# Ulixes-8/UNet-Implementations

Hardware: AMD Instinct MI355X
Metric: images/sec (512x512, bs/GPU=8) Our_UNet train step (higher is better)
Workload: dtype f32; 1 GPU; Our_UNet 6-stage 3-class 512x512 bs=8/GPU fp32 train step (fwd + Dice/wCE loss + bwd + SGD-Nesterov), train mode, HIP conv/IN/upsample kernels; global_batch=8, parallelism=dp1, world=1

## Files before the change

### include/unet_hip.h

```cpp
#ifndef UNET_HIP_H_
#define UNET_HIP_H_

#include <stddef.h>
#include <stdint.h>

#ifdef __cplusplus
extern "C" {
#endif

#define UNET_ABI_VERSION 11

#define UNET_OK 0
#define UNET_E_INVALID (-1)
#define UNET_E_LAUNCH (-2)
#define UNET_E_WORKSPACE (-3)

typedef void* unet_stream_t;

const char* unet_last_error(void);
int unet_abi_version(void);
int unet_device_count(void);

int unet_debug_set_chunk_limit(int64_t bytes);

// ... 222 lines not shown
int unet_conv3x3_up_bwd_data(const float* D, const float* wd, int Cin_total, int ci_offset,
                             float* g, int N, int h, int w, int Cout, int Ccols, int accumulate,
                             unet_stream_t stream);

typedef struct unet_bwd_stats {
  const float* y;
  const float* mean;
  const float* rstd;
  const float* gamma;
  const float* beta;
  const float* mask;
  float slope;
  void* partial;
  size_t partial_bytes;
  int tiles_out;
} unet_bwd_stats;
int unet_conv3x3_bwd_data_bs(const float* dy, const float* wd, int Cin_total, int ci_offset,
                             float* dx, int N, int H, int W, int Cout, int Ccols, int stride,
                             int accumulate, unet_bwd_stats* bs, unet_stream_t stream);
int unet_conv3x3_bwd_data_bs_b16(const uint16_t* dy, const float* wd, int Cin_total, int ci_offset,
                                 uint16_t* dx, int N, int H, int W, int Cout, int Ccols, int stride,
                                 int accumulate, unet_bwd_stats* bs, unet_stream_t stream);
int unet_conv3x3_bwd_data_bs_bf16x3(const float* dy, const float* wd, const uint16_t* wd3,
                                    int Cin_total, int ci_offset, float* dx, int N, int H, int W,
                                    int Cout, int Ccols, int stride, int accumulate,
                                    unet_bwd_stats* bs, unet_stream_t stream);
int unet_conv3x3_up_bwd_data_bs(const float* D, const float* wd, int Cin_total, int ci_offset,
                                float* g, int N, int h, int w, int Cout, int Ccols, int accumulate,
                                unet_bwd_stats* bs, unet_stream_t stream);
int unet_conv_wino_supported(int N, int H, int W, int C0, int C1, int Cout);
int unet_set_c32_winograd(int on);
// ... 27 lines not shown
int unet_instnorm_lrelu_drop_bwd_partials(const float* ga, const float* y, const float* mean,
                                          const float* rstd, const float* gamma,
                                          const float* beta, const float* mask, float slope,
                                          float* dy, float* dgamma, float* dbeta, float* dbias,
                                          const void* partial, int tiles, void* workspace,
                                          size_t workspace_bytes, int N, int HW, int C,
                                          unet_stream_t stream);
int unet_instnorm_lrelu_drop_bwd_partials_b16(const uint16_t* ga, const uint16_t* y,
                                              const float* mean, const float* rstd,
                                              const float* gamma, const float* beta,
                                              const float* mask, float slope, uint16_t* dy,
                                              float* dgamma, float* dbeta, float* dbias,
                                              const void* partial, int tiles, void* workspace,
                                              size_t workspace_bytes, int N, int HW, int C,
                                              unet_stream_t stream);

int unet_conv_in_fwd_b16(const unet_act_src* s0, const unet_act_src* s1, float slope,
                         const float* w, const float* bias, int ksize, int stride, uint16_t* y,
                         void* workspace, size_t workspace_bytes, int* stats_px_out, int N, int H,
                         int W, int Cout, unet_stream_t stream);
int unet_conv_in_fwd_b16_wb(const unet_act_src* s0, const unet_act_src* s1, float slope,
                            const float* w, const uint16_t* wb, const float* bias, int ksize,
                            int stride, uint16_t* y, void* workspace, size_t workspace_bytes,
                            int* stats_px_out, int N, int H, int W, int Cout, unet_stream_t stream);
int unet_conv3x3_bwd_data_bs_b16_wb(const uint16_t* dy, const float* wd, const uint16_t* wdb,
                                    int Cin_total, int ci_offset, uint16_t* dx, int N, int H,
                                    int W, int Cout, int Ccols, int stride, int accumulate,
                                    unet_bwd_stats* bs, unet_stream_t stream);
int unet_conv_in_stats_finalize_b16(const uint16_t* y, void* workspace, size_t workspace_bytes,
                                    int stats_px, const float* gamma, const float* beta, float eps,
// ... 97 lines not shown
```

### unet-implementations_amd/_lib.py

```python
import ctypes
import os
import subprocess

_HERE = os.path.dirname(os.path.abspath(__file__))
LIB_PATH = os.environ.get("UNET_HIP_LIB") or os.path.join(_HERE, "libunet_hip.so")
CSRC = os.path.join(_HERE, "csrc")

ABI_VERSION = 11

_c = ctypes
_p = _c.c_void_p
_i = _c.c_int
_f = _c.c_float
_sz = _c.c_size_t
_i64 = _c.c_int64



class ActSrc(ctypes.Structure):
    _fields_ = [("x", _p), ("C", _i), ("alpha", _p), ("beta", _p)]


_ps = _c.POINTER(ActSrc)


class BwdStats(ctypes.Structure):
    _fields_ = [("y", _p), ("mean", _p), ("rstd", _p), ("gamma", _p), ("beta", _p), ("mask", _p),
                ("slope", _f), ("partial", _p), ("partial_bytes", _sz), ("tiles_out", _i)]


_pbs = _c.POINTER(BwdStats)

SIGNATURES = {
    "unet_last_error": (_c.c_char_p, []),
    "unet_abi_version": (_i, []),
    "unet_device_count": (_i, []),
    "unet_debug_set_chunk_limit": (_i, [_i64]),
    "unet_debug_record_launches": (_i, [_i]),
    "unet_debug_recorded_launches": (_sz, [_p, _sz]),
    "unet_nchw_to_nhwc": (_i, [_p, _p, _i, _i, _i, _i, _p]),
    "unet_nhwc_to_nchw": (_i, [_p, _p, _i, _i, _i, _i, _p]),
    "unet_pack_conv3x3_weights": (_i, [_p, _p, _p, _i, _i, _p]),
    "unet_conv3x3_fwd": (_i, [_p, _i, _p, _i, _p, _p, _p, _i, _i, _i, _i, _i, _p]),
# ... 74 lines not shown
    "unet_conv3x3_bwd_weight_is_winograd": (_i, [_i, _i, _i, _i, _i, _i]),
    "unet_conv_up_wino_supported": (_i, [_i, _i, _i, _i, _i, _i]),
    "unet_conv_up_in_fwd_wino": (_i, [_ps, _ps, _f, _p, _p, _p, _p, _sz, _c.POINTER(_i), _i, _i,
                                      _i, _i, _p]),
    "unet_conv3x3_bwd_data_bs_wino": (_i, [_p, _p, _i, _i, _p, _i, _i, _i, _i, _i, _pbs, _p]),
    "unet_conv3x3_bwd_data_bs_b16": (_i, [_p, _p, _i, _i, _p, _i, _i, _i, _i, _i, _i, _i, _pbs, _p]),
    "unet_conv3x3_bwd_data_bs_b16_wb": (_i, [_p, _p, _p, _i, _i, _p, _i, _i, _i, _i, _i, _i, _i, _pbs,
                                             _p]),
    "unet_conv3x3_bwd_data_bs_bf16x3": (_i, [_p, _p, _p, _i, _i, _p, _i, _i, _i, _i, _i, _i, _i, _pbs,
                                             _p]),
    "unet_conv3x3_up_bwd_data_bs": (_i, [_p, _p, _i, _i, _p, _i, _i, _i, _i, _i, _i, _pbs, _p]),
    "unet_instnorm_lrelu_drop_bwd_partials": (_i, [_p, _p, _p, _p, _p, _p, _p, _f, _p, _p, _p, _p,
                                                   _p, _i, _p, _sz, _i, _i, _i, _p]),
    "unet_instnorm_lrelu_drop_bwd_partials_b16": (_i, [_p, _p, _p, _p, _p, _p, _p, _f, _p, _p, _p, _p,
                                                       _p, _i, _p, _sz, _i, _i, _i, _p]),
    "unet_conv_in_fwd_b16": (_i, [_ps, _ps, _f, _p, _p, _i, _i, _p, _p, _sz, _c.POINTER(_i), _i, _i,
                                  _i, _i, _p]),
    "unet_conv_in_fwd_b16_wb": (_i, [_ps, _ps, _f, _p, _p, _p, _i, _i, _p, _p, _sz, _c.POINTER(_i),
                                     _i, _i, _i, _i, _p]),
    "unet_conv_in_stats_finalize_b16": (_i, [_p, _p, _sz, _i, _p, _p, _f, _p, _p, _p, _p, _p, _i, _i,
                                             _i, _p]),
    "unet_conv_in_bwd_weight_b16": (_i, [_ps, _f, _p, _p, _i, _i, _i, _i, _p, _sz, _i, _i, _i, _i,
                                         _p]),
    "unet_conv3x3_bwd_data_b16": (_i, [_p, _p, _i, _i, _p, _i, _i, _i, _i, _i, _i, _i, _p]),
    "unet_instnorm_lrelu_drop_bwd_b16": (_i, [_p, _p, _p, _p, _p, _p, _p, _f, _p, _p, _p, _p, _p,
                                              _sz, _i, _i, _i, _p]),
    "unet_upsample2x_in_fwd_b16": (_i, [_ps, _f, _p, _i, _i, _i, _p]),
    "unet_upsample2x_bwd_taps_b16": (_i, [_p, _p, _i, _i, _i, _i, _p]),
    "unet_conv3x3_up_bwd_weight_b16": (_i, [_ps, _f, _p, _p, _i, _i, _p, _sz, _i, _i, _i, _i, _p]),
    "unet_conv_up_in_fwd_b16_supported": (_i, [_i, _i, _i, _i, _i, _i]),
# ... 74 lines not shown
```

### unet-implementations_amd/csrc/common.h

```cpp
#pragma once
#include <hip/hip_runtime.h>
#include <stdarg.h>
#include <stdint.h>
#include <stdio.h>

#include "../../include/unet_hip.h"

typedef float f32x4 __attribute__((ext_vector_type(4)));
typedef float f32x16 __attribute__((ext_vector_type(16)));
typedef __bf16 bf16x8 __attribute__((ext_vector_type(8)));
typedef __bf16 bf16x4 __attribute__((ext_vector_type(4)));

void unet_set_error(const char* fmt, ...);

#define UNET_REQUIRE(cond, ...)        \
  do {                                 \
    if (!(cond)) {                     \
      unet_set_error(__VA_ARGS__);     \
      return UNET_E_INVALID;           \
    }                                  \
  } while (0)

#define UNET_CHECK_LAUNCH(name)                                              \
  do {                                                                       \
// ... 134 lines not shown
  }
  return v;
}

__device__ __forceinline__ void wf_merge(float& n, float& mean, float& m2, float nb, float mb,
                                         float m2b) {
  if (nb == 0.f) return;
  const float nt = n + nb;
  const float d = mb - mean;
  const float f = nb / nt;
  mean += d * f;
  m2 += m2b + d * d * n * f;
  n = nt;
}

#endif
```

### unet-implementations_amd/csrc/conv_igemm.hip

```cpp
#include "conv_params.h"

namespace unet_conv {
namespace {


template <int BM, int BN, int WM, int WN, int BK, bool FUSED = false, int KG = 1>
__global__ __launch_bounds__(256 * KG, KG == 1 ? 2 : 1) void conv_igemm_kernel(const IgemmParams p) {
  constexpr int LDA = BK + 4;
  constexpr int SEGS = BK / 4;
  constexpr int ROWS = 256 / SEGS;
  constexpr int TM = WM / 32, TN = WN / 32;
  constexpr int WAVES_N = BN / WN;
  static_assert((BM / WM) * (BN / WN) == 4, "4 waves per block");
  constexpr int A_PASSES = BM / ROWS;
  constexpr int B_PASSES = BN / ROWS;
  constexpr int A_TILE = BM * LDA, B_TILE = BN * LDA;
  extern __shared__ __attribute__((aligned(16))) float smem[];
  const int grp = KG > 1 ? __builtin_amdgcn_readfirstlane((int)(threadIdx.x >> 8)) : 0;
  const bool lead = KG == 1 || grp == 0;
  float* As = smem + grp * 2 * (A_TILE + B_TILE);
  float* Bs = As + 2 * A_TILE;

  const int tid = threadIdx.x & 255, lane = tid & 63, wave = tid >> 6;
  const int li = lane & 31, lh = lane >> 5;
// ... 1279 lines not shown

extern "C" int unet_conv3x3_fwd_bf16x3(const float* x0, int C0, const float* x1, int C1,
                                       const float* wf, const uint16_t* wf3, const float* bias,
                                       float* y, int N, int H, int W, int Cout, int stride,
                                       unet_stream_t stream) {
  return conv3x3_fwd_impl(x0, C0, x1, C1, wf, bias, y, N, H, W, Cout, stride, C0 == 3 ? 0 : 3,
                          (hipStream_t)stream, wf3);
}

static int conv3x3_bwd_data_impl(const float* dy, const float* wd, int Cin_total, int ci_offset,
                                 float* dx, int N, int H, int W, int Cout, int Ccols, int stride,
                                 int accumulate, int prec, hipStream_t stream,
                                 const uint16_t* wd3 = nullptr, int b16 = 0,
                                 unet_bwd_stats* bs = nullptr) {
  const long long es = b16 ? 2 : 4;
  if (bs) bs->tiles_out = 0;
  if (prec == 3 && bs && stride == 2) prec = 0;
  const bool use_bs = bs && (prec == 0 || prec == 3 || b16) && bs->y && bs->mean &&
                      bs->rstd && bs->gamma &&
                      bs->beta && bs->partial &&
                      bs->partial_bytes >= (size_t)N * ceil_div(H * W, 64) * Ccols * sizeof(float2);
  UNET_REQUIRE(dy && wd && dx, "conv3x3_bwd_data: null pointer");
  UNET_REQUIRE(prec != 3 || wd3, "conv3x3_bwd_data_bf16x3: the pre-split weight planes are null");
  UNET_REQUIRE(stride == 1 || stride == 2, "conv3x3_bwd_data: stride %d unsupported", stride);
  UNET_REQUIRE(Cout > 0 && Cout % 32 == 0 && Ccols > 0 && Ccols % 32 == 0 && ci_offset >= 0 &&
                   ci_offset + Ccols <= Cin_total,
               "conv3x3_bwd_data: bad channel counts Cout=%d Ccols=%d slice %d of %d", Cout, Ccols,
               ci_offset, Cin_total);
  UNET_REQUIRE(stride == 1 || (H % 2 == 0 && W % 2 == 0),
               "conv3x3_bwd_data: stride 2 needs even H, W");
// ... 59 lines not shown
    else if (rf_applicable(p) && (Cout == 32 || !patch_f32_applicable(p) || p.Hin % 8 != 0))
      rc = (Cout == 32) ? launch_igemm_rf<128, 32, 32, 32, true>(p, 1, stream, &bs_px)
                        : launch_igemm_rf<128, 32, 32, 32, false>(p, 1, stream, &bs_px);
    else
      rc = dispatch_igemm(p, stream, nullptr, use_bs ? &bs_px : nullptr);
    if (rc == UNET_OK && use_bs && bs_px > 0) bs->tiles_out = H * W / bs_px;
    return rc;
  }
  p.Hl = H / 2; p.Wl = W / 2; p.sout = 2;
  {
    const long long tiles = ceil_div64((long long)N * p.Hl * p.Wl, 128) * (Ccols / 32);
    if (prec == 0 && !b16) {
      IgemmParams q = p;
      if (!use_bs) q.bs_partial = nullptr;
      int bt = 0;
      const int rc = launch_dgrad_s2_patch_auto(q, stream, &bt);
      if (rc != 1) {
        if (rc == UNET_OK && use_bs && bt > 0) bs->tiles_out = bt;
        return rc;
      }
    }
    if (b16) {
      IgemmParams q = p;
      if (!use_bs) q.bs_partial = nullptr;
      int bt = 0;
      const int rc = launch_dgrad_s2_patch_b16_auto(q, stream, use_bs ? &bt : nullptr);
      if (rc != 1) {
        if (rc == UNET_OK && use_bs && bt > 0) bs->tiles_out = bt;
        return rc;
      }
      p.bs_partial = nullptr;
// ... 653 lines not shown
```

### unet-implementations_amd/csrc/conv_params.h

```cpp
#pragma once
#include "common.h"

namespace unet_conv {

struct IgemmParams {
  const float* src0;
  const float* src1;
  int C0, C1;
  const float* w;
  int tap_stride;
  int n_off;
  unsigned src0_bytes, src1_bytes, w_bytes;
  const float* bias;
  float* out;
  int ldo;
  int accumulate;
  int N, Hin, Win;
  int Hl, Wl;
  int Hout, Wout;
  int sin;
  int sout, py, px;
  int ntaps;
  unsigned tapw[3];
  int Ncols;
// ... 4 lines not shown
  const float* act1_alpha; const float* act1_beta;
  float slope;
  float2* stats;
  int stats_tiles;
  int tap_cstride;
  int src0_pitch;
  const float* bs_y;
  const float* bs_mean;
  const float* bs_rstd;
  const float* bs_gamma;
  const float* bs_beta;
  const float* bs_mask;
  float2* bs_partial;
  int bs_tiles;
  int bs_tile0;
};

long long& chunk_limit_bytes();
inline int batch_chunk(int N, long long per_image_bytes) {
  const long long lim = chunk_limit_bytes();
  const long long n = lim / (per_image_bytes > 0 ? per_image_bytes : 1);
  return (int)(n < N ? n : N);
}

inline void set_tap(IgemmParams& p, int t, int oy, int ox, int wt) {
  const unsigned e = (unsigned)(oy + 1) | ((unsigned)(ox + 1) << 2) | ((unsigned)wt << 4);
  p.tapw[t >> 2] |= e << ((t & 3) * 8);
}

#ifdef __HIPCC__
template <typename TO>
// ... 98 lines not shown
    }
  s1 += __shfl_xor(s1, 32, 64);
  s2 += __shfl_xor(s2, 32, 64);
  return float2{s1, s2};
}
template <int BN, int WAVES_M>
__device__ __forceinline__ bool block_col_sums(float2* red, float2& out) {
  __syncthreads();
  const int c = threadIdx.x;
  if (c >= BN) return false;
  float a = red[c].x, b = red[c].y;
#pragma unroll
  for (int k = 1; k < WAVES_M; ++k) { a += red[k * BN + c].x; b += red[k * BN + c].y; }
  out = float2{a, b};
  return true;
}

template <int BN, int WAVES_M>
__device__ __forceinline__ bool block_col_stats(float2* red, int wave_m, int col_local, bool writer,
                                                float2 mine, float cnt_wave, float2& out) {
  if (writer) red[wave_m * BN + col_local] = mine;
  __syncthreads();
  const int c = threadIdx.x;
  if (c >= BN) return false;
  float mean = red[c].x, m2 = red[c].y;
  if (WAVES_M == 2) {
    wf_merge_eq(mean, m2, red[BN + c].x, red[BN + c].y, cnt_wave);
  } else if (WAVES_M == 4) {
    float mean1 = red[2 * BN + c].x, m21 = red[2 * BN + c].y;
    wf_merge_eq(mean, m2, red[BN + c].x, red[BN + c].y, cnt_wave);
// ... 5 lines not shown
}
#endif

bool patch_f32_applicable(const IgemmParams& p);
int launch_patch_f32_auto(const IgemmParams& p, hipStream_t stream,
                          int* stats_px = nullptr, int* bs_px = nullptr);
int launch_patch_up_auto(const IgemmParams& p, hipStream_t stream, int* stats_px);
int& c32_winograd_flag();
bool c32_applicable(const IgemmParams& p);
int launch_c32(const IgemmParams& p, int fused, hipStream_t stream, int* tile_px);
bool wino_up32_applicable(const IgemmParams& p);
int launch_wino_up32(const IgemmParams& p, hipStream_t stream);
bool patch_s2_applicable(const IgemmParams& p);
int launch_patch_s2_auto(const IgemmParams& p, hipStream_t stream, int* stats_px);
int launch_patch_s2_b16_auto(const IgemmParams& p, hipStream_t stream, int* stats_px);
int launch_dgrad_s2_patch_auto(const IgemmParams& p, hipStream_t stream, int* bs_tiles_out);
int launch_patch_b16_up_auto(const IgemmParams& p, hipStream_t stream, int* stats_px);
int launch_dgrad_s2_patch_b16_auto(const IgemmParams& p, hipStream_t stream, int* bs_tiles_out);
int launch_patch_split_auto(const IgemmParams& p, hipStream_t stream);
int launch_patch_b16_auto(const IgemmParams& p, hipStream_t stream, int* stats_px,
                          int* bs_px = nullptr);
int launch_patch_split_fused_auto(const IgemmParams& p, hipStream_t stream, int* stats_px,
                                  int* bs_px);
bool patch_split_applicable(const IgemmParams& p);
int dispatch_igemm(const IgemmParams& p, hipStream_t stream,
                   int* stats_px = nullptr, int* bs_px = nullptr);
int dispatch_igemm_bf16(const IgemmParams& p, hipStream_t stream);
int dispatch_igemm_b16(const IgemmParams& p, hipStream_t stream, int* stats_px,
                       int* bs_px = nullptr);
int dispatch_igemm_split(const IgemmParams& p, hipStream_t stream);

// ... 2 lines not shown
```

### unet-implementations_amd/csrc/conv_patch.hip

```cpp
#include "conv_params.h"

#include <utility>

namespace unet_conv {
namespace {

template <int B, int... I, typename F>
__device__ __forceinline__ void for_range_p_impl(std::integer_sequence<int, I...>, F&& f) {
  (f(std::integral_constant<int, B + I>{}), ...);
}
template <int B, int E, typename F>
__device__ __forceinline__ void for_range_p(F&& f) {
  for_range_p_impl<B>(std::make_integer_sequence<int, (E > B ? E - B : 0)>{}, f);
}

template <int BN, int WM, int WN, int TH, bool ACT = false, bool STATS = false, bool BSTATS = false>
__global__ __launch_bounds__(256, 2) void conv_patch_split_kernel(const IgemmParams p) {
  constexpr int LDA = 24;
  constexpr int TW = 32, PW = TW + 2;
  constexpr int PPIX = (TH + 2) * PW;
  constexpr int P_PLANE = PPIX * LDA;
  constexpr int P_SLOTS = PPIX * 4;
  constexpr int P_PASSES = (P_SLOTS + 255) / 256;
  constexpr int B_SLOTS = BN * 6, B_PASSES = (B_SLOTS + 255) / 256;
// ... 1355 lines not shown
          }
        }
      }
  }
  if (p.bs_partial) {
    float2* red = reinterpret_cast<float2*>(Ps);
    static_assert(WAVES_M * BN * 2 <= PPIX * LDA, "reduction scratch fits in the patch area");
#pragma unroll
    for (int nb = 0; nb < TN; ++nb) {
      const float a = s1[nb] + __shfl_xor(s1[nb], 32, 64);
      const float b = s2[nb] + __shfl_xor(s2[nb], 32, 64);
      if (lh == 0) red[(wave / WAVES_N) * BN + wn0 + nb * 32 + li] = float2{a, b};
    }
    float2 out;
    if (block_col_sums<BN, WAVES_M>(red, out))
      p.bs_partial[((size_t)n * p.bs_tiles + ty * tiles_x + tx) * p.Ncols + n0 + tid] = out;
  }
}

template <int BN, int WM, int WN, int TH, bool WB = false>
__global__ __launch_bounds__(256, 2) void conv_dgrad_s2_patch_b16_kernel(const IgemmParams p) {
  constexpr int BK = 32, LDA = BK + 8;
  constexpr int TW = 32, PW = TW + 1, PH = TH + 1;
  constexpr int PPIX = PH * PW;
  constexpr int P_SLOTS = PPIX * 8;
  constexpr int P_PASSES = (P_SLOTS + 255) / 256;
  constexpr int B_SEGS = WB ? 4 : 8;
  constexpr int B_SETS = WB ? 2 : 1;
  constexpr int B_SLOTS = 3 * BN * B_SEGS, B_PASSES = (B_SLOTS + 255) / 256;
  constexpr int B_TILE = 3 * BN * LDA;
  constexpr int TM = WM / 32, TN = WN / 32;
// ... 585 lines not shown
  p.bs_tile0 = 0;
  if (!bs_tiles_out) p.bs_partial = nullptr;
  if (nc % 64 == 0 && p.Hl % 4 == 0 && pos / 128 * (nc / 64) >= 256) {
    p.bs_tiles = p.Hl * p.Wl / 128;
    if (bs_tiles_out) *bs_tiles_out = p.bs_partial ? p.bs_tiles : 0;
    return launch_dgrad_s2_patch_b16<64, 32, 64, 4>(p, stream);
  }
  if (nc == 32 && p.Hl % 8 == 0 && pos / 256 >= 256) {
    p.bs_tiles = p.Hl * p.Wl / 256;
    if (bs_tiles_out) *bs_tiles_out = p.bs_partial ? p.bs_tiles : 0;
    return launch_dgrad_s2_patch_b16<32, 64, 32, 8>(p, stream);
  }
  return 1;
}

int launch_dgrad_s2_patch_auto(const IgemmParams& p0, hipStream_t stream, int* bs_tiles_out) {
  IgemmParams p = p0;
  if (p.Wl % 32 != 0 || p.C0 % 32 != 0 || p.Hout != 2 * p.Hl || p.Wout != 2 * p.Wl) return 1;
  const long long pos = (long long)p.N * p.Hl * p.Wl;
  const int nc = p.Ncols;
  p.bs_tile0 = 0;
  if (nc % 64 == 0 && p.Hl % 4 == 0 && pos / 128 * (nc / 64) >= 256) {
    p.bs_tiles = p.Hl * p.Wl / 128;
    if (bs_tiles_out) *bs_tiles_out = p.bs_partial ? p.bs_tiles : 0;
    return launch_dgrad_s2_patch<64, 32, 64, 4>(p, stream);
  }
  if (nc == 32 && p.Hl % 8 == 0 && pos / 256 >= 256) {
    p.bs_tiles = p.Hl * p.Wl / 256;
    if (bs_tiles_out) *bs_tiles_out = p.bs_partial ? p.bs_tiles : 0;
    return launch_dgrad_s2_patch<32, 64, 32, 8>(p, stream);
  }
  return 1;
}

bool patch_s2_applicable(const IgemmParams& p) {
  IgemmParams std_taps{};
  for (int t = 0; t < 9; ++t) set_tap(std_taps, t, t / 3 - 1, t % 3 - 1, t);
  return p.ntaps == 9 && p.tap_cstride == 0 && p.src0_pitch == 0 && p.sin == 2 &&
         p.sout == 1 && p.Hin == 2 * p.Hl && p.Win == 2 * p.Wl && p.Hl == p.Hout &&
         p.Wl == p.Wout && p.Hl % 4 == 0 && p.Wl % 32 == 0 && p.C0 % 16 == 0 && p.C1 % 16 == 0 &&
         !p.accumulate && p.tapw[0] == std_taps.tapw[0] && p.tapw[1] == std_taps.tapw[1] &&
         p.tapw[2] == std_taps.tapw[2];
}

// ... 285 lines not shown
```

### unet-implementations_amd/csrc/conv_wino.hip

```cpp
#include "conv_params.h"
#include "lds_asm.h"
#include <utility>

namespace unet_conv {
namespace {

typedef int i32x4v __attribute__((ext_vector_type(4)));
template <int I> using wn_ic = std::integral_constant<int, I>;
template <int B, int... I, typename F>
__device__ __forceinline__ void wn_for_impl(std::integer_sequence<int, I...>, F&& f) {
  (f(wn_ic<B + I>{}), ...);
}
template <int B, int E, typename F>
__device__ __forceinline__ void wn_for(F&& f) {
  wn_for_impl<B>(std::make_integer_sequence<int, E - B>{}, f);
}

constexpr int WN_TH = 8, WN_TW = 32;
constexpr int WN_PW = WN_TW + 2, WN_PH = WN_TH + 2;
constexpr int WN_PPIX = WN_PH * WN_PW;
constexpr int WN_BN = 64;
constexpr int WN_KC = 8;
constexpr int WN_RP = 360;
constexpr int WN_BUF = 16 * 64 * WN_KC;
// ... 400 lines not shown
#pragma unroll
        for (int q = 0; q < 4; ++q) {
          const size_t pix = ((size_t)n * H + oy + (q >> 1)) * W + ox + 2 * r + (q & 1);
          const float y = p.bs_y[pix * p.ldo + col];
          const float z = fmaf(y, cf.A, cf.B0);
          const float gz = yv[b][r][q] * cf.mk * (z > 0.f ? 1.f : p.slope);
          s1 += gz;
          s2 = fmaf(gz, (y - cf.mu) * cf.rs, s2);
        }
      s1 += __shfl_xor(s1, 16, 64); s2 += __shfl_xor(s2, 16, 64);
      s1 += __shfl_xor(s1, 32, 64); s2 += __shfl_xor(s2, 32, 64);
      if (fk_e == 0) red[tg_e * WN_BN + 32 * nh_e + 16 * b + fm_e] = float2{s1, s2};
    }
    float2 out;
    if (block_col_sums<WN_BN, 4>(red, out))
      p.bs_partial[((size_t)n * p.bs_tiles + ty * tiles_x + tx) * p.Ncols + n0 + tid] = out;
  }
}

__device__ __forceinline__ void wino_pack_items(const float* __restrict__ w,
                                                float* __restrict__ uf, float* __restrict__ ud,
                                                int Cout, int Cin, int dir, long long block) {
  float* dst = dir == 0 ? uf : ud;
  if (!dst) return;
  const int Nn = dir == 0 ? Cout : Cin, Kt = dir == 0 ? Cin : Cout;
  const int kchunks = Kt / WN_KC;
  const long long items = (long long)Nn * kchunks;
  const long long idx = block * 256 + threadIdx.x;
  if (idx >= items) return;
  const int nl = (int)(idx & 63);
  const long long rest = idx >> 6;
// ... 179 lines not shown
               "conv3x3_bwd_data_bs_wino: bad channel slice");
  UNET_REQUIRE(wino_shape_ok(N, H, W, Cout, 0, Ccols, ci_offset),
               "conv3x3_bwd_data_bs_wino: shape N=%d %dx%d %d->%d not tiled by the Winograd kernel",
               N, H, W, Cout, Ccols);
  WinoParams wp{};
  IgemmParams& p = wp.g;
  p.src0 = dy; p.C0 = Cout; p.C1 = 0;
  p.src0_bytes = (unsigned)((long long)N * H * W * Cout * 4);
  p.n_off = ci_offset;
  p.out = dx; p.ldo = Ccols; p.N = N; p.Hin = p.Hl = p.Hout = H; p.Win = p.Wl = p.Wout = W;
  p.Ncols = Ccols;
  wp.wu = ud;
  const bool use_bs = bs && bs->y && bs->mean && bs->rstd && bs->gamma && bs->beta &&
                      bs->partial &&
                      bs->partial_bytes >= (size_t)N * (H * W / 256) * Ccols * sizeof(float2);
  if (bs) bs->tiles_out = 0;
  if (use_bs) {
    p.bs_y = bs->y; p.bs_mean = bs->mean; p.bs_rstd = bs->rstd; p.bs_gamma = bs->gamma;
    p.bs_beta = bs->beta; p.bs_mask = bs->mask; p.slope = bs->slope;
    p.bs_partial = reinterpret_cast<float2*>(bs->partial);
    p.bs_tiles = H * W / 256; p.bs_tile0 = 0;
    bs->tiles_out = p.bs_tiles;
    return launch_wino<false, false, true>(wp, (hipStream_t)stream);
  }
  return launch_wino<false, false, false>(wp, (hipStream_t)stream);
}
```

### unet-implementations_amd/csrc/instnorm.hip

```cpp
#include "common.h"

namespace {

constexpr int kThreads = 256;
constexpr int kColsumChunks = 32;

__host__ __device__ inline int split_for(int N, int HW, int C) {
  int ppi = kThreads / (C / 4);
  if (ppi < 1) ppi = 1;
  int max_split = HW / (ppi * 8);
  if (max_split < 1) max_split = 1;
  int want = (2048 + N - 1) / N;
  int s = want < max_split ? want : max_split;
  return s < 1 ? 1 : s;
}

template <typename TS>
__global__ __launch_bounds__(kThreads) void in_stats_kernel(const TS* __restrict__ y,
                                                            float2* __restrict__ partial, int HW,
                                                            int C, int split) {
  extern __shared__ __attribute__((aligned(16))) float smem[];
  const int lpp = C >> 2;
  const int groups = kThreads / lpp;
  const int tid = threadIdx.x;
// ... 47 lines not shown
  float* sm_m2 = sm_mean + groups * C;
  if (grp < groups) {
    sm_cnt[grp * lpp + c4] = cnt;
    *reinterpret_cast<f32x4*>(sm_mean + grp * C + c4 * 4) = mean;
    *reinterpret_cast<f32x4*>(sm_m2 + grp * C + c4 * 4) = m2;
  }
  __syncthreads();
  for (int c = tid; c < C; c += kThreads) {
    float n0 = 0.f, mu = 0.f, q = 0.f;
    for (int g = 0; g < groups; ++g)
      wf_merge(n0, mu, q, sm_cnt[g * lpp + (c >> 2)], sm_mean[g * C + c], sm_m2[g * C + c]);
    partial[((size_t)n * split + s) * C + c] = float2{mu, q};
  }
}

constexpr int FL = 32;
__global__ __launch_bounds__(32 * FL) void in_stats_finalize_kernel(
    const float2* __restrict__ partial, const float* __restrict__ gamma,
    const float* __restrict__ beta, float eps, const float* __restrict__ mask,
    float* __restrict__ mean, float* __restrict__ rstd, float* __restrict__ alpha,
    float* __restrict__ beta2, int N, int HW, int C, int split) {
  __shared__ float sn[FL][33], sm[FL][33], sq[FL][33];
  const int cl = threadIdx.x & 31, l = threadIdx.x >> 5;
  const int c = blockIdx.x * 32 + cl, n = blockIdx.y;
  const int per = (HW + split - 1) / split;
  float cnt = 0.f, mu = 0.f, q = 0.f;
  if (c < C) {
    for (int s = l; s < split; s += FL) {
      const int pb = s * per;
      int pe = pb + per;
      if (pe > HW) pe = HW;
// ... 206 lines not shown
  __syncthreads();
  for (int c = tid; c < C; c += kThreads) {
    float a = 0.f, b = 0.f;
    for (int g = 0; g < groups; ++g) {
      a += sm1[g * C + c];
      b += sm2[g * C + c];
    }
    partial[((size_t)n * split + s) * C + c] = float2{a, b};
  }
}

__global__ __launch_bounds__(32 * FL) void in_bwd_finalize1_kernel(const float2* __restrict__ partial,
                                                               float2* __restrict__ coef,
                                                               float2* __restrict__ sums, int HW,
                                                               int C, int split) {
  __shared__ double sa[FL][33], sb[FL][33];
  const int cl = threadIdx.x & 31, l = threadIdx.x >> 5;
  const int c = blockIdx.x * 32 + cl, n = blockIdx.y;
  double da_ = 0.0, db_ = 0.0;
  if (c < C)
    for (int s = l; s < split; s += FL) {
      const float2 v = partial[((size_t)n * split + s) * C + c];
      da_ += (double)v.x;
      db_ += (double)v.y;
    }
  sa[l][cl] = da_; sb[l][cl] = db_;
  __syncthreads();
  if (l == 0 && c < C) {
    da_ = 0.0; db_ = 0.0;
#pragma unroll 4
    for (int k = 0; k < FL; ++k) { da_ += sa[k][cl]; db_ += sb[k][cl]; }
    float a = (float)da_, b = (float)db_;
    const float inv = 1.f / (float)HW;
    coef[(size_t)n * C + c] = float2{a * inv, b * inv};
    sums[(size_t)n * C + c] = float2{a, b};
  }
}

template <typename TS>
__global__ __launch_bounds__(kThreads) void in_bwd_apply_kernel(
    const TS* ga , const TS* __restrict__ y, const float* __restrict__ mean,
    const float* __restrict__ rstd, const float* __restrict__ gamma,
    const float* __restrict__ beta, const float* __restrict__ mask, float slope,
    const float2* __restrict__ coef, TS* dy, float* __restrict__ dbias_partial,
    int HW, int C, int split, const float2* __restrict__ sums, float* __restrict__ dgamma,
    float* __restrict__ dbeta, float* __restrict__ dbias) {
  extern __shared__ __attribute__((aligned(16))) float smem[];
  const int lpp = C >> 2;
  const int groups = kThreads / lpp;
  const int tid = threadIdx.x;
  const int grp = tid / lpp, c4 = tid - grp * lpp;
// ... 197 lines not shown

extern "C" int unet_instnorm_lrelu_drop_bwd_partials_b16(
    const uint16_t* ga, const uint16_t* y, const float* mean, const float* rstd,
    const float* gamma, const float* beta, const float* mask, float slope, uint16_t* dy,
    float* dgamma, float* dbeta, float* dbias, const void* partial, int tiles, void* workspace,
    size_t workspace_bytes, int N, int HW, int C, unet_stream_t stream) {
  UNET_REQUIRE(partial && tiles > 0, "instnorm_lrelu_drop_bwd_partials_b16: no summaries");
  return instnorm_bwd_impl<__bf16>(reinterpret_cast<const __bf16*>(ga),
                                   reinterpret_cast<const __bf16*>(y), mean, rstd, gamma, beta,
                                   mask, slope, reinterpret_cast<__bf16*>(dy), dgamma, dbeta, dbias,
                                   workspace, workspace_bytes, N, HW, C, (hipStream_t)stream,
                                   reinterpret_cast<const float2*>(partial), tiles);
}

template <typename TS>
static int instnorm_bwd_impl(const TS* ga, const TS* y, const float* mean, const float* rstd,
                             const float* gamma, const float* beta, const float* mask, float slope,
                             TS* dy, float* dgamma, float* dbeta, float* dbias, void* workspace,
                             size_t workspace_bytes, int N, int HW, int C, hipStream_t stream,
                             const float2* ext_partial, int ext_tiles) {
  UNET_REQUIRE(ga && y && mean && rstd && gamma && beta && dy && workspace,
               "instnorm_lrelu_drop_bwd: null pointer");
  UNET_REQUIRE(shape_ok(N, HW, C) && kThreads % (C / 4) == 0,
               "instnorm_lrelu_drop_bwd: unsupported shape N=%d HW=%d C=%d", N, HW, C);
  if (workspace_bytes < unet_instnorm_workspace_bytes(N, HW, C)) {
    unet_set_error("instnorm_lrelu_drop_bwd: workspace too small");
    return UNET_E_WORKSPACE;
  }
  const int split = split_for(N, HW, C);
  const int groups = kThreads / (C / 4);
// ... 31 lines not shown
```

### unet-implementations_amd/ops.py

```python
import ctypes
import functools
import struct
import threading

import torch

from ._lib import ActSrc, BwdStats, check, lib


_raw_stream = getattr(torch._C, "_cuda_getCurrentRawStream", None)
_raw_device = getattr(torch._C, "_cuda_getDevice", None)


def _stream():
    if _raw_stream is not None and _raw_device is not None:
        return _raw_stream(_raw_device())
    return torch.cuda.current_stream().cuda_stream


class KernelTimer:

    def __init__(self, only=None):
        self.only = only
        self.records = []
# ... 84 lines not shown
    return getattr(lib(), name)


@functools.lru_cache(maxsize=None)
def _twin(name, b16):
    return getattr(lib(), name + "_b16" if b16 else name)


def _call_nxt(fn, args, nxt):
    if nxt is None:
        check(fn(*args, None, _stream()))
        return
    bs = nxt.c_struct()
    check(fn(*args, ctypes.byref(bs), _stream()))
    nxt.tiles = bs.tiles_out


_defer = threading.local()


def _wgrad_ws(nbytes, like):
    ws = _ws(nbytes, like)
    held = getattr(_defer, "held", None)
    if held is not None:
        held.append(ws)
    return ws


class wgrad_deferral:

# ... 172 lines not shown
    assert wf.shape[0] == 9 and wf.shape[2] == C0 + C1
    Ho, Wo = (H - 1) // stride + 1, (W - 1) // stride + 1
    y = out if out is not None else _f32((N, Ho, Wo, Cout), x0)
    fn, planes, tag = _sel_conv3x3_fwd(_prec(bf16), C0)
    if planes and wf3 is None:
        raise ValueError("bf16x3 needs wf3 from pack_conv3x3_weights_bf16x3")
    w3 = (_ptr(wf3),) if planes else ()
    t0 = _begin("conv")
    check(fn(_ptr(x0), C0, _ptr(x1), C1, _ptr(wf), *w3, _ptr(bias), _ptr(y), N, H, W, Cout, stride,
             _stream()))
    if t0 is not None:
        _timer.end(tag, 2.0 * N * Ho * Wo * 9 * (C0 + C1) * Cout, 1, t0)
    return y


class NextNorm:

    __slots__ = ("y", "st", "gamma", "beta", "mask", "slope", "partial", "tiles")

    def __init__(self, y, st, gamma, beta, mask, slope):
        self.y, self.st, self.gamma, self.beta, self.mask, self.slope = y, st, gamma, beta, mask, slope
        self.partial, self.tiles = None, 0

    def c_struct(self):
        N, H, W, C = self.y.shape
        nbytes = N * ((H * W + 63) // 64) * C * 8
        self.partial = torch.empty(nbytes, dtype=torch.uint8, device=self.y.device)
        return BwdStats(_ptr(self.y), _ptr(self.st[0]), _ptr(self.st[1]), _ptr(self.gamma),
                        _ptr(self.beta), _ptr(self.mask), self.slope, _ptr(self.partial), nbytes, 0)


def _c32_winograd(N, H, W, Cin, Cout, stride):
    return bool(lib().unet_conv_c32_is_winograd(N, H, W, Cin, Cout, stride))


_c32_override = None


def c32_winograd_override():
    return _c32_override


class c32_winograd_scope:

# ... 126 lines not shown
    check(lib().unet_instnorm_stats(_ptr(y), _ptr(gamma), _ptr(beta), eps, _ptr(st[0]),
                                    _ptr(st[1]), _ptr(st[2]), _ptr(st[3]), _ptr(ws), ws.numel(), N,
                                    H * W, C, _stream()))
    return st


def instnorm_lrelu_drop_fwd(y, alpha, beta2, mask, slope, out=None):
    N, H, W, C = y.shape
    a = out if out is not None else torch.empty_like(y)
    check(lib().unet_instnorm_lrelu_drop_fwd(_ptr(y), _ptr(alpha), _ptr(beta2), _ptr(mask), slope,
                                             _ptr(a), N, H * W, C, _stream()))
    return a


def instnorm_lrelu_drop_bwd(ga, y, mean, rstd, gamma, beta, mask, slope, dgamma, dbeta, dbias,
                            out=None, partials=None):
    N, H, W, C = y.shape
    dy = ga if out is None else out
    ws = _ws(lib().unet_instnorm_workspace_bytes(N, H * W, C), y)
    if partials is not None:
        name, part, launches, passes = "unet_instnorm_lrelu_drop_bwd_partials", \
            (_ptr(partials[0]), partials[1]), 2, 3.0
    else:
        name, part, launches, passes = "unet_instnorm_lrelu_drop_bwd", (), 5, 5
        if _is_b16(y) != _is_b16(ga):
            raise TypeError("ga and y must share their storage type")
    t0 = _begin()
    check(_twin(name, _is_b16(y))(
        _ptr(ga), _ptr(y), _ptr(mean), _ptr(rstd), _ptr(gamma), _ptr(beta), _ptr(mask), slope,
        _ptr(dy), _ptr(dgamma), _ptr(dbeta), _ptr(dbias), *part, _ptr(ws), ws.numel(), N, H * W, C,
        _stream()))
    if t0 is not None:
        _timer.end("instnorm_bwd", 0.0, launches, t0, nbytes=y.element_size() * passes * y.numel())
    return dy
# ... 664 lines not shown
```

Baseline: 468.7 images/s.

## Finalize instance-norm backward partial sums inside the dgrad kernel via last-workgroup counter

The stride-2 patch dgrad and Winograd dgrad kernels now store per-tile IN backward partial sums with atomic stores. The last workgroup per column block, found through an atomic ticket counter, reduces those partials into coef/sums inside the same kernel. The IN backward then runs a single apply kernel instead of a separate finalize launch plus apply. This removes one kernel launch and one pass over the partials per norm layer, at the cost of a persistent counter buffer, extra LDS and a serialized reduction in the last workgroup.

```diff
diff --git a/include/unet_hip.h b/include/unet_hip.h
--- a/include/unet_hip.h
+++ b/include/unet_hip.h
@@ -260,7 +260,12 @@
   void* partial;
   size_t partial_bytes;
   int tiles_out;
+  void* coef;
+  void* counters;
+  size_t counters_bytes;
+  int finalized_out;
 } unet_bwd_stats;
+#define UNET_BWD_STATS_FINALIZE 0x46494e31
 int unet_conv3x3_bwd_data_bs(const float* dy, const float* wd, int Cin_total, int ci_offset,
                              float* dx, int N, int H, int W, int Cout, int Ccols, int stride,
                              int accumulate, unet_bwd_stats* bs, unet_stream_t stream);
@@ -318,6 +323,19 @@
                                               const void* partial, int tiles, void* workspace,
                                               size_t workspace_bytes, int N, int HW, int C,
                                               unet_stream_t stream);
+int unet_instnorm_lrelu_drop_bwd_finalized(const float* ga, const float* y, const float* mean,
+                                           const float* rstd, const float* gamma,
+                                           const float* beta, const float* mask, float slope,
+                                           float* dy, float* dgamma, float* dbeta, float* dbias,
+                                           const void* coef_sums, int N, int HW, int C,
+                                           unet_stream_t stream);
+int unet_instnorm_lrelu_drop_bwd_finalized_b16(const uint16_t* ga, const uint16_t* y,
+                                               const float* mean, const float* rstd,
+                                               const float* gamma, const float* beta,
+                                               const float* mask, float slope, uint16_t* dy,
+                                               float* dgamma, float* dbeta, float* dbias,
+                                               const void* coef_sums, int N, int HW, int C,
+                                               unet_stream_t stream);
 
 int unet_conv_in_fwd_b16(const unet_act_src* s0, const unet_act_src* s1, float slope,
                          const float* w, const float* bias, int ksize, int stride, uint16_t* y,
diff --git a/unet-implementations_amd/_lib.py b/unet-implementations_amd/_lib.py
--- a/unet-implementations_amd/_lib.py
+++ b/unet-implementations_amd/_lib.py
@@ -26,7 +26,8 @@
 
 class BwdStats(ctypes.Structure):
     _fields_ = [("y", _p), ("mean", _p), ("rstd", _p), ("gamma", _p), ("beta", _p), ("mask", _p),
-                ("slope", _f), ("partial", _p), ("partial_bytes", _sz), ("tiles_out", _i)]
+                ("slope", _f), ("partial", _p), ("partial_bytes", _sz), ("tiles_out", _i),
+                ("coef", _p), ("counters", _p), ("counters_bytes", _sz), ("finalized_out", _i)]
 
 
 _pbs = _c.POINTER(BwdStats)
@@ -131,6 +132,10 @@
                                                    _p, _i, _p, _sz, _i, _i, _i, _p]),
     "unet_instnorm_lrelu_drop_bwd_partials_b16": (_i, [_p, _p, _p, _p, _p, _p, _p, _f, _p, _p, _p, _p,
                                                        _p, _i, _p, _sz, _i, _i, _i, _p]),
+    "unet_instnorm_lrelu_drop_bwd_finalized": (_i, [_p, _p, _p, _p, _p, _p, _p, _f, _p, _p, _p, _p,
+                                                    _p, _i, _i, _i, _p]),
+    "unet_instnorm_lrelu_drop_bwd_finalized_b16": (_i, [_p, _p, _p, _p, _p, _p, _p, _f, _p, _p, _p,
+                                                        _p, _p, _i, _i, _i, _p]),
     "unet_conv_in_fwd_b16": (_i, [_ps, _ps, _f, _p, _p, _i, _i, _p, _p, _sz, _c.POINTER(_i), _i, _i,
                                   _i, _i, _p]),
     "unet_conv_in_fwd_b16_wb": (_i, [_ps, _ps, _f, _p, _p, _p, _i, _i, _p, _p, _sz, _c.POINTER(_i),
diff --git a/unet-implementations_amd/csrc/common.h b/unet-implementations_amd/csrc/common.h
--- a/unet-implementations_amd/csrc/common.h
+++ b/unet-implementations_amd/csrc/common.h
@@ -172,4 +172,76 @@
   n = nt;
 }
 
+__device__ __forceinline__ void st_summary(float2* dst, const float2 v) {
+  const unsigned long long bits =
+      ((unsigned long long)__float_as_uint(v.y) << 32) | (unsigned long long)__float_as_uint(v.x);
+  __hip_atomic_store(reinterpret_cast<unsigned long long*>(dst), bits, __ATOMIC_RELAXED,
+                     __HIP_MEMORY_SCOPE_AGENT);
+}
+template <bool COHERENT>
+__device__ __forceinline__ float2 ld_summary(const float2* src) {
+  if constexpr (COHERENT) {
+    const unsigned long long bits =
+        __hip_atomic_load(reinterpret_cast<const unsigned long long*>(src), __ATOMIC_RELAXED,
+                          __HIP_MEMORY_SCOPE_AGENT);
+    return float2{__uint_as_float((unsigned)bits), __uint_as_float((unsigned)(bits >> 32))};
+  } else {
+    return *src;
+  }
+}
+__device__ __forceinline__ bool finalize_by_last_workgroup(unsigned* counter, unsigned expected,
+                                                           unsigned* flag, int writers) {
+  if ((int)threadIdx.x < writers) asm volatile("s_waitcnt vmcnt(0)" ::: "memory");
+  __syncthreads();
+  if (threadIdx.x == 0) {
+    const unsigned ticket =
+        __hip_atomic_fetch_add(counter, 1u, __ATOMIC_RELAXED, __HIP_MEMORY_SCOPE_AGENT);
+    const bool last = ticket + 1u == expected;
+    if (last) __hip_atomic_store(counter, 0u, __ATOMIC_RELAXED, __HIP_MEMORY_SCOPE_AGENT);
+    *flag = last ? 1u : 0u;
+  }
+  __syncthreads();
+  const bool last = *flag != 0u;
+  __builtin_amdgcn_fence(__ATOMIC_ACQUIRE, "wavefront");
+  return last;
+}
+
+constexpr int kFinLanes = 32;
+template <int T, bool COHERENT>
+__device__ __forceinline__ void in_bwd_finalize1_body(const float2* partial, float2* coef,
+                                                      float2* sums, int HW, int C, int split,
+                                                      int n, int cg, double* sa, double* sb) {
+  const int cl = threadIdx.x & 31;
+  const int c = cg * 32 + cl;
+  for (int l = threadIdx.x >> 5; l < kFinLanes; l += T / 32) {
+    double da_ = 0.0, db_ = 0.0;
+    if (c < C)
+      for (int s = l; s < split; s += 4 * kFinLanes) {
+        float2 v[4];
+#pragma unroll
+        for (int j = 0; j < 4; ++j)
+          if (s + j * kFinLanes < split)
+            v[j] = ld_summary<COHERENT>(partial + ((size_t)n * split + s + j * kFinLanes) * C + c);
+#pragma unroll
+        for (int j = 0; j < 4; ++j)
+          if (s + j * kFinLanes < split) {
+            da_ += (double)v[j].x;
+            db_ += (double)v[j].y;
+          }
+      }
+    sa[l * 32 + cl] = da_; sb[l * 32 + cl] = db_;
+  }
+  __syncthreads();
+  if (threadIdx.x < 32 && c < C) {
+    double da_ = 0.0, db_ = 0.0;
+#pragma unroll 4
+    for (int k = 0; k < kFinLanes; ++k) { da_ += sa[k * 32 + cl]; db_ += sb[k * 32 + cl]; }
+    float a = (float)da_, b = (float)db_;
+    const float inv = 1.f / (float)HW;
+    coef[(size_t)n * C + c] = float2{a * inv, b * inv};
+    sums[(size_t)n * C + c] = float2{a, b};
+  }
+  __syncthreads();
+}
+
 #endif
diff --git a/unet-implementations_amd/csrc/conv_igemm.hip b/unet-implementations_amd/csrc/conv_igemm.hip
--- a/unet-implementations_amd/csrc/conv_igemm.hip
+++ b/unet-implementations_amd/csrc/conv_igemm.hip
@@ -1317,6 +1317,7 @@
                                  const uint16_t* wd3 = nullptr, int b16 = 0,
                                  unet_bwd_stats* bs = nullptr) {
   const long long es = b16 ? 2 : 4;
+  unet_bwd_stats* const bs_fin = bs_finalize_requested(bs);
   if (bs) bs->tiles_out = 0;
   if (prec == 3 && bs && stride == 2) prec = 0;
   const bool use_bs = bs && (prec == 0 || prec == 3 || b16) && bs->y && bs->mean &&
@@ -1406,7 +1407,7 @@
       IgemmParams q = p;
       if (!use_bs) q.bs_partial = nullptr;
       int bt = 0;
-      const int rc = launch_dgrad_s2_patch_auto(q, stream, &bt);
+      const int rc = launch_dgrad_s2_patch_auto(q, stream, &bt, use_bs ? bs_fin : nullptr);
       if (rc != 1) {
         if (rc == UNET_OK && use_bs && bt > 0) bs->tiles_out = bt;
         return rc;
diff --git a/unet-implementations_amd/csrc/conv_params.h b/unet-implementations_amd/csrc/conv_params.h
--- a/unet-implementations_amd/csrc/conv_params.h
+++ b/unet-implementations_amd/csrc/conv_params.h
@@ -42,7 +42,29 @@
   float2* bs_partial;
   int bs_tiles;
   int bs_tile0;
+  unsigned* bs_counter;
+  float2* bs_coef;
+  float2* bs_sums;
+  int bs_HW;
 };
+
+constexpr int kFinalizeInKernelMaxTiles = 256;
+
+inline unet_bwd_stats* bs_finalize_requested(unet_bwd_stats* bs) {
+  return bs && bs->tiles_out == UNET_BWD_STATS_FINALIZE ? bs : nullptr;
+}
+inline void bs_finalize_setup(IgemmParams& p, unet_bwd_stats* bs, int HW, int BN) {
+  p.bs_counter = nullptr;
+  if (bs) bs->finalized_out = 0;
+  if (!bs || !p.bs_partial || !bs->coef || !bs->counters) return;
+  if (p.bs_tiles < 1 || p.bs_tiles > kFinalizeInKernelMaxTiles || p.Ncols % BN) return;
+  if (bs->counters_bytes < (size_t)p.N * (p.Ncols / BN) * sizeof(unsigned)) return;
+  p.bs_counter = reinterpret_cast<unsigned*>(bs->counters);
+  p.bs_coef = reinterpret_cast<float2*>(bs->coef);
+  p.bs_sums = p.bs_coef + (size_t)p.N * p.Ncols;
+  p.bs_HW = HW;
+  bs->finalized_out = 1;
+}
 
 long long& chunk_limit_bytes();
 inline int batch_chunk(int N, long long per_image_bytes) {
@@ -171,6 +193,23 @@
   for (int k = 1; k < WAVES_M; ++k) { a += red[k * BN + c].x; b += red[k * BN + c].y; }
   out = float2{a, b};
   return true;
+}
+
+constexpr size_t kBsFinalizeLds = 16 + 2 * kFinLanes * 32 * sizeof(double);
+template <int T, int BN>
+__device__ __forceinline__ void bs_finalize_in_kernel(const IgemmParams& p, int n, int n0,
+                                                      void* lds) {
+  if (!p.bs_counter) return;
+  unsigned* flag = reinterpret_cast<unsigned*>(lds);
+  double* sa = reinterpret_cast<double*>(reinterpret_cast<char*>(lds) + 16);
+  double* sb = sa + kFinLanes * 32;
+  if (!finalize_by_last_workgroup(p.bs_counter + (size_t)n * (p.Ncols / BN) + n0 / BN,
+                                  (unsigned)p.bs_tiles, flag, BN))
+    return;
+#pragma unroll 1
+  for (int g = 0; g < BN / 32; ++g)
+    in_bwd_finalize1_body<T, true>(p.bs_partial, p.bs_coef, p.bs_sums, p.bs_HW, p.Ncols,
+                                   p.bs_tiles, n, n0 / 32 + g, sa, sb);
 }
 
 template <int BN, int WAVES_M>
@@ -206,7 +245,8 @@
 bool patch_s2_applicable(const IgemmParams& p);
 int launch_patch_s2_auto(const IgemmParams& p, hipStream_t stream, int* stats_px);
 int launch_patch_s2_b16_auto(const IgemmParams& p, hipStream_t stream, int* stats_px);
-int launch_dgrad_s2_patch_auto(const IgemmParams& p, hipStream_t stream, int* bs_tiles_out);
+int launch_dgrad_s2_patch_auto(const IgemmParams& p, hipStream_t stream, int* bs_tiles_out,
+                               unet_bwd_stats* bs = nullptr);
 int launch_patch_b16_up_auto(const IgemmParams& p, hipStream_t stream, int* stats_px);
 int launch_dgrad_s2_patch_b16_auto(const IgemmParams& p, hipStream_t stream, int* bs_tiles_out);
 int launch_patch_split_auto(const IgemmParams& p, hipStream_t stream);
diff --git a/unet-implementations_amd/csrc/conv_patch.hip b/unet-implementations_amd/csrc/conv_patch.hip
--- a/unet-implementations_amd/csrc/conv_patch.hip
+++ b/unet-implementations_amd/csrc/conv_patch.hip
@@ -1393,7 +1393,9 @@
     }
     float2 out;
     if (block_col_sums<BN, WAVES_M>(red, out))
-      p.bs_partial[((size_t)n * p.bs_tiles + ty * tiles_x + tx) * p.Ncols + n0 + tid] = out;
+      st_summary(p.bs_partial + ((size_t)n * p.bs_tiles + ty * tiles_x + tx) * p.Ncols + n0 + tid, out);
+    static_assert(kBsFinalizeLds <= PPIX * LDA * sizeof(float), "finalize scratch fits in the patch area");
+    bs_finalize_in_kernel<256, BN>(p, n, n0, smem);
   }
 }
 
@@ -2009,7 +2011,8 @@
   return 1;
 }
 
-int launch_dgrad_s2_patch_auto(const IgemmParams& p0, hipStream_t stream, int* bs_tiles_out) {
+int launch_dgrad_s2_patch_auto(const IgemmParams& p0, hipStream_t stream, int* bs_tiles_out,
+                               unet_bwd_stats* bs) {
   IgemmParams p = p0;
   if (p.Wl % 32 != 0 || p.C0 % 32 != 0 || p.Hout != 2 * p.Hl || p.Wout != 2 * p.Wl) return 1;
   const long long pos = (long long)p.N * p.Hl * p.Wl;
@@ -2018,11 +2021,13 @@
   if (nc % 64 == 0 && p.Hl % 4 == 0 && pos / 128 * (nc / 64) >= 256) {
     p.bs_tiles = p.Hl * p.Wl / 128;
     if (bs_tiles_out) *bs_tiles_out = p.bs_partial ? p.bs_tiles : 0;
+    bs_finalize_setup(p, bs, p.Hout * p.Wout, 64);
     return launch_dgrad_s2_patch<64, 32, 64, 4>(p, stream);
   }
   if (nc == 32 && p.Hl % 8 == 0 && pos / 256 >= 256) {
     p.bs_tiles = p.Hl * p.Wl / 256;
     if (bs_tiles_out) *bs_tiles_out = p.bs_partial ? p.bs_tiles : 0;
+    bs_finalize_setup(p, bs, p.Hout * p.Wout, 32);
     return launch_dgrad_s2_patch<32, 64, 32, 8>(p, stream);
   }
   return 1;
diff --git a/unet-implementations_amd/csrc/conv_wino.hip b/unet-implementations_amd/csrc/conv_wino.hip
--- a/unet-implementations_amd/csrc/conv_wino.hip
+++ b/unet-implementations_amd/csrc/conv_wino.hip
@@ -438,7 +438,8 @@
     }
     float2 out;
     if (block_col_sums<WN_BN, 4>(red, out))
-      p.bs_partial[((size_t)n * p.bs_tiles + ty * tiles_x + tx) * p.Ncols + n0 + tid] = out;
+      st_summary(p.bs_partial + ((size_t)n * p.bs_tiles + ty * tiles_x + tx) * p.Ncols + n0 + tid, out);
+    bs_finalize_in_kernel<512, WN_BN>(p, n, n0, smem);
   }
 }
 
@@ -648,6 +649,7 @@
   const bool use_bs = bs && bs->y && bs->mean && bs->rstd && bs->gamma && bs->beta &&
                       bs->partial &&
                       bs->partial_bytes >= (size_t)N * (H * W / 256) * Ccols * sizeof(float2);
+  unet_bwd_stats* const bs_fin = bs_finalize_requested(bs);
   if (bs) bs->tiles_out = 0;
   if (use_bs) {
     p.bs_y = bs->y; p.bs_mean = bs->mean; p.bs_rstd = bs->rstd; p.bs_gamma = bs->gamma;
@@ -655,6 +657,7 @@
     p.bs_partial = reinterpret_cast<float2*>(bs->partial);
     p.bs_tiles = H * W / 256; p.bs_tile0 = 0;
     bs->tiles_out = p.bs_tiles;
+    bs_finalize_setup(p, bs_fin, H * W, WN_BN);
     return launch_wino<false, false, true>(wp, (hipStream_t)stream);
   }
   return launch_wino<false, false, false>(wp, (hipStream_t)stream);
diff --git a/unet-implementations_amd/csrc/instnorm.hip b/unet-implementations_amd/csrc/instnorm.hip
--- a/unet-implementations_amd/csrc/instnorm.hip
+++ b/unet-implementations_amd/csrc/instnorm.hip
@@ -85,7 +85,7 @@
   }
 }
 
-constexpr int FL = 32;
+constexpr int FL = kFinLanes;
 __global__ __launch_bounds__(32 * FL) void in_stats_finalize_kernel(
     const float2* __restrict__ partial, const float* __restrict__ gamma,
     const float* __restrict__ beta, float eps, const float* __restrict__ mask,
@@ -322,27 +322,9 @@
                                                                float2* __restrict__ coef,
                                                                float2* __restrict__ sums, int HW,
                                                                int C, int split) {
-  __shared__ double sa[FL][33], sb[FL][33];
-  const int cl = threadIdx.x & 31, l = threadIdx.x >> 5;
-  const int c = blockIdx.x * 32 + cl, n = blockIdx.y;
-  double da_ = 0.0, db_ = 0.0;
-  if (c < C)
-    for (int s = l; s < split; s += FL) {
-      const float2 v = partial[((size_t)n * split + s) * C + c];
-      da_ += (double)v.x;
-      db_ += (double)v.y;
-    }
-  sa[l][cl] = da_; sb[l][cl] = db_;
-  __syncthreads();
-  if (l == 0 && c < C) {
-    da_ = 0.0; db_ = 0.0;
-#pragma unroll 4
-    for (int k = 0; k < FL; ++k) { da_ += sa[k][cl]; db_ += sb[k][cl]; }
-    float a = (float)da_, b = (float)db_;
-    const float inv = 1.f / (float)HW;
-    coef[(size_t)n * C + c] = float2{a * inv, b * inv};
-    sums[(size_t)n * C + c] = float2{a, b};
-  }
+  __shared__ double sa[FL * 32], sb[FL * 32];
+  in_bwd_finalize1_body<32 * FL, false>(partial, coef, sums, HW, C, split, blockIdx.y, blockIdx.x,
+                                        sa, sb);
 }
 
 template <typename TS>
@@ -570,6 +552,50 @@
 }
 
 template <typename TS>
+static int instnorm_bwd_apply_impl(const TS* ga, const TS* y, const float* mean, const float* rstd,
+                                   const float* gamma, const float* beta, const float* mask,
+                                   float slope, TS* dy, float* dgamma, float* dbeta, float* dbias,
+                                   const void* coef_sums, int N, int HW, int C,
+                                   hipStream_t stream) {
+  UNET_REQUIRE(ga && y && mean && rstd && gamma && beta && dy && coef_sums,
+               "instnorm_lrelu_drop_bwd_finalized: null pointer");
+  UNET_REQUIRE(shape_ok(N, HW, C) && kThreads % (C / 4) == 0,
+               "instnorm_lrelu_drop_bwd_finalized: unsupported shape N=%d HW=%d C=%d", N, HW, C);
+  const int split = split_for(N, HW, C);
+  const int groups = kThreads / (C / 4);
+  const float2* coef = reinterpret_cast<const float2*>(coef_sums);
+  const float2* sums = coef + (size_t)N * C;
+  const size_t lds1 = (size_t)groups * C * sizeof(float);
+  hipLaunchKernelGGL(in_bwd_apply_kernel<TS>, dim3(split, N), dim3(kThreads), lds1, stream, ga, y, mean,
+                     rstd, gamma, beta, mask, slope, coef, dy, (float*)nullptr, HW, C, split, sums,
+                     dgamma, dbeta, dbias);
+  UNET_CHECK_LAUNCH("in_bwd_apply");
+  return UNET_OK;
+}
+
+extern "C" int unet_instnorm_lrelu_drop_bwd_finalized(const float* ga, const float* y,
+                                                      const float* mean, const float* rstd,
+                                                      const float* gamma, const float* beta,
+                                                      const float* mask, float slope, float* dy,
+                                                      float* dgamma, float* dbeta, float* dbias,
+                                                      const void* coef_sums, int N, int HW, int C,
+                                                      unet_stream_t stream) {
+  return instnorm_bwd_apply_impl<float>(ga, y, mean, rstd, gamma, beta, mask, slope, dy, dgamma,
+                                        dbeta, dbias, coef_sums, N, HW, C, (hipStream_t)stream);
+}
+
+extern "C" int unet_instnorm_lrelu_drop_bwd_finalized_b16(
+    const uint16_t* ga, const uint16_t* y, const float* mean, const float* rstd,
+    const float* gamma, const float* beta, const float* mask, float slope, uint16_t* dy,
+    float* dgamma, float* dbeta, float* dbias, const void* coef_sums, int N, int HW, int C,
+    unet_stream_t stream) {
+  return instnorm_bwd_apply_impl<__bf16>(reinterpret_cast<const __bf16*>(ga),
+                                         reinterpret_cast<const __bf16*>(y), mean, rstd, gamma,
+                                         beta, mask, slope, reinterpret_cast<__bf16*>(dy), dgamma,
+                                         dbeta, dbias, coef_sums, N, HW, C, (hipStream_t)stream);
+}
+
+template <typename TS>
 static int instnorm_bwd_impl(const TS* ga, const TS* y, const float* mean, const float* rstd,
                              const float* gamma, const float* beta, const float* mask, float slope,
                              TS* dy, float* dgamma, float* dbeta, float* dbias, void* workspace,
diff --git a/unet-implementations_amd/ops.py b/unet-implementations_amd/ops.py
--- a/unet-implementations_amd/ops.py
+++ b/unet-implementations_amd/ops.py
@@ -122,6 +122,8 @@
     bs = nxt.c_struct()
     check(fn(*args, ctypes.byref(bs), _stream()))
     nxt.tiles = bs.tiles_out
+    if bs.finalized_out:
+        nxt.partial = FinalizedSums(nxt.coef)
 
 
 _defer = threading.local()
@@ -324,20 +326,49 @@
     return y
 
 
+_COUNTER_WORDS = 16384
+_BWD_STATS_FINALIZE = 0x46494e31
+_counters = {}
+
+
+def _finalize_counters(dev):
+    buf = _counters.get(dev)
+    if buf is None:
+        if torch.cuda.is_current_stream_capturing():
+            return None
+        buf = _counters[dev] = torch.zeros(4 * _COUNTER_WORDS, dtype=torch.uint8, device=dev)
+    return buf
+
+
+class FinalizedSums:
+
+    __slots__ = ("coef",)
+
+    def __init__(self, coef):
+        self.coef = coef
+
+
 class NextNorm:
 
-    __slots__ = ("y", "st", "gamma", "beta", "mask", "slope", "partial", "tiles")
+    __slots__ = ("y", "st", "gamma", "beta", "mask", "slope", "partial", "tiles", "coef",
+                 "in_kernel")
 
     def __init__(self, y, st, gamma, beta, mask, slope):
         self.y, self.st, self.gamma, self.beta, self.mask, self.slope = y, st, gamma, beta, mask, slope
-        self.partial, self.tiles = None, 0
+        self.partial, self.tiles, self.coef = None, 0, None
+        self.in_kernel = True
 
     def c_struct(self):
         N, H, W, C = self.y.shape
         nbytes = N * ((H * W + 63) // 64) * C * 8
         self.partial = torch.empty(nbytes, dtype=torch.uint8, device=self.y.device)
+        cnt = _finalize_counters(self.y.device) if self.in_kernel and N * C <= 32 * _COUNTER_WORDS \
+            else None
+        self.coef = _f32((2, N, C, 2), self.y) if cnt is not None else None
         return BwdStats(_ptr(self.y), _ptr(self.st[0]), _ptr(self.st[1]), _ptr(self.gamma),
-                        _ptr(self.beta), _ptr(self.mask), self.slope, _ptr(self.partial), nbytes, 0)
+                        _ptr(self.beta), _ptr(self.mask), self.slope, _ptr(self.partial), nbytes,
+                        _BWD_STATS_FINALIZE if cnt is not None else 0,
+                        _ptr(self.coef), _ptr(cnt), 0 if cnt is None else cnt.numel(), 0)
 
 
 def _c32_winograd(N, H, W, Cin, Cout, stride):
@@ -494,10 +525,21 @@
 
 
 def instnorm_lrelu_drop_bwd(ga, y, mean, rstd, gamma, beta, mask, slope, dgamma, dbeta, dbias,
-                            out=None, partials=None):
+                            out=None, partials=None, keep_ws=None):
     N, H, W, C = y.shape
     dy = ga if out is None else out
     ws = _ws(lib().unet_instnorm_workspace_bytes(N, H * W, C), y)
+    if keep_ws is not None:
+        keep_ws.append(ws)
+    if partials is not None and isinstance(partials[0], FinalizedSums):
+        t0 = _begin()
+        check(_twin("unet_instnorm_lrelu_drop_bwd_finalized", _is_b16(y))(
+            _ptr(ga), _ptr(y), _ptr(mean), _ptr(rstd), _ptr(gamma), _ptr(beta), _ptr(mask), slope,
+            _ptr(dy), _ptr(dgamma), _ptr(dbeta), _ptr(dbias), _ptr(partials[0].coef), N, H * W, C,
+            _stream()))
+        if t0 is not None:
+            _timer.end("instnorm_bwd", 0.0, 1, t0, nbytes=y.element_size() * 3.0 * y.numel())
+        return dy
     if partials is not None:
         name, part, launches, passes = "unet_instnorm_lrelu_drop_bwd_partials", \
             (_ptr(partials[0]), partials[1]), 2, 3.0
```

Result: no change. 468.7 images/s (median of 2 runs) (-0.0%).
